# microsoft/SpeechT5

Hardware: AMD Instinct MI355X
Metric: audio-sec/s fwd+bwd SpeechT5-Base (higher is better)
Workload: dtype bf16

## Files before the change

### include/speecht5_hip.h

```cpp
#ifndef SPEECHT5_HIP_H
#define SPEECHT5_HIP_H
#include <stdint.h>
#ifdef __cplusplus
extern "C" {
#endif

#define ST5_F32 0
#define ST5_BF16 1

#define ST5_ACT_NONE 0
#define ST5_ACT_GELU 1
#define ST5_ACT_RELU 2
#define ST5_ACT_TANH 3
#define ST5_ACT_LRELU_01 4
#define ST5_ACT_LRELU_001 5

#define ST5_GEMM_A_KSTRIDED 1
#define ST5_GEMM_B_KSTRIDED 2
#define ST5_GEMM_OUT_F32 4
#define ST5_GEMM_DACT 8
#define ST5_GEMM_DEFERRABLE 16

typedef struct st5_operand {
  const void* ptr;
// ... 44 lines not shown
int st5_gemm_set_mx8_heavy_nk(int nk);
int st5_quant_mxfp8(const void* x, int64_t ld, void* q, int64_t q_ld, uint8_t* s, int64_t s_ld, int64_t rows, int32_t cols, void* stream);
int st5_multi_quant_mxfp8(const void* jobs, int32_t njobs, int32_t nblocks, void* stream);
int st5_gemm_tn_group(const st5_gemm_params* list, int32_t n, int dtype, void* stream);
int st5_gemm_set_tn_group_tile(int mode);
int st5_gemm_tn_group_is_phased(int32_t M, int32_t N, int32_t K);
int st5_gemm_defer_splitk(int enabled, void* stream);
int st5_gemm_flush_splitk(void* stream);

int st5_layernorm_fwd(const void* x, const float* gamma, const float* beta, void* y, float* mean,
                      float* rstd, int64_t rows, int32_t cols, float eps, int dtype, void* stream);
int st5_layernorm_bwd(const void* dy, const void* x, const float* gamma, const float* mean, const float* rstd, void* dx,
                      float* dgamma, float* dbeta, void* ws, int64_t rows, int32_t cols,
                      void* dx_dropped ,
                      float drop_p, uint64_t drop_seed, int dtype, void* stream);
int st5_layernorm_fwd_q8(const void* x, const float* gamma, const float* beta, void* y, float* mean, float* rstd, void* q, uint8_t* sc,
                         int64_t rows, int32_t cols, float eps, void* stream);
int st5_layernorm_bwd_add(const void* dy, const void* x, const float* gamma, const float* mean, const float* rstd, void* dx, float* dgamma,
                          float* dbeta, void* ws, int64_t rows, int32_t cols, const void* addend, int dtype, void* stream);
int st5_layernorm_gelu_fwd(const void* x, const float* gamma, const float* beta, void* y, float* mean, float* rstd, int64_t rows, int32_t cols,
                           float eps, int dtype, void* stream);
int st5_layernorm_gelu_bwd(const void* dy, const void* x, const float* gamma, const float* beta, const float* mean, const float* rstd, void* dx,
                           float* dgamma, float* dbeta, void* ws, int64_t rows, int32_t cols, int dtype, void* stream);
int st5_layernorm_gated_fwd(const void* x, const float* gamma, const float* beta, void* y, float* mean, float* rstd, int64_t rows,
                            int32_t cols, float eps, const float* keep, const void* skip, int dtype, void* stream);
int st5_layernorm_gated_bwd(const void* dy, const void* x, const float* gamma, const float* mean, const float* rstd, void* dx,
                            float* dgamma, float* dbeta, void* ws, int64_t rows, int32_t cols, void* dx_dropped, float drop_p,
                            uint64_t drop_seed, const float* keep, int dtype, void* stream);
int st5_layernorm_fwd_gate(const void* x, const float* gamma, const float* beta, void* y, float* mean, float* rstd, int64_t rows,
                           int32_t cols, float eps, const float* keep, const void* skip, const float* gate, int dtype, void* stream);
int st5_layernorm_bwd_gate(const void* dy, const void* x, const float* gamma, const float* mean, const float* rstd, void* dx, float* dgamma,
                           float* dbeta, void* ws, int64_t rows, int32_t cols, void* dx_dropped, float drop_p, uint64_t drop_seed,
                           const float* keep, const float* gate, int dtype, void* stream);
int st5_layernorm_defer(int enabled, void* stream);
int st5_layernorm_flush(void* stream);
int64_t st5_layernorm_bwd_ws_bytes(int64_t rows, int32_t cols);

int st5_softmax_fwd(const void* scores, const void* qp, const uint8_t* kpm, void* probs, void* probs_drop,
                    int32_t BH, int32_t H, int32_t T, int32_t S, int32_t lds, int32_t nb, int32_t maxrel,
                    int32_t causal, float dropout_p, uint64_t seed, int dtype, void* stream);
int st5_softmax_bwd(void* dP_inout, const void* probs, const float* dP_extra, void* dqp, int32_t BH, int32_t T,
                    int32_t S, int32_t lds, int32_t nb, int32_t maxrel, float dropout_p, uint64_t seed, int dtype,
                    void* stream);

int st5_flash_attn_fwd(const void* q, int64_t q_ld, const void* k, int64_t k_ld, const void* v, int64_t v_ld, void* o,
                       int64_t o_ld, float* lse, const void* pe, const uint8_t* kpm, int32_t B, int32_t H, int32_t T,
                       int32_t S, int32_t head_dim, int32_t nb, int32_t maxrel, int32_t causal, int32_t lds, float scale,
                       float dropout_p, uint64_t seed, int dtype, void* stream);

int32_t st5_flash_attn_qp_row(int32_t nb);
int st5_flash_attn_qp_table(const void* q, int64_t q_ld, const void* pe, void* qp_out, int32_t B, int32_t H, int32_t T, int32_t nb,
                            float scale, int dtype, void* stream);
int st5_flash_attn_set_impl(int impl);

int st5_flash_attn_fwd_qp(const void* q, int64_t q_ld, const void* k, int64_t k_ld, const void* v, int64_t v_ld, void* o,
                          int64_t o_ld, float* lse, const void* pe, const uint8_t* kpm, int32_t B, int32_t H, int32_t T,
                          int32_t S, int32_t head_dim, int32_t nb, int32_t maxrel, int32_t causal, int32_t lds, float scale,
                          float dropout_p, uint64_t seed, void* qp_out, int dtype, void* stream);

int st5_flash_attn_fwd_qp_gate(const void* q, int64_t q_ld, const void* k, int64_t k_ld, const void* v, int64_t v_ld, void* o,
                               int64_t o_ld, float* lse, const void* pe, const uint8_t* kpm, int32_t B, int32_t H, int32_t T,
                               int32_t S, int32_t head_dim, int32_t nb, int32_t maxrel, int32_t causal, int32_t lds, float scale,
                               float dropout_p, uint64_t seed, void* qp_out, const float* gate, int dtype, void* stream);

int st5_flash_attn_bwd(const void* q, int64_t q_ld, const void* k, int64_t k_ld, const void* v, int64_t v_ld, const void* o,
                       int64_t o_ld, const void* dout, int64_t do_ld, void* dq, int64_t dq_ld, void* dk, int64_t dk_ld, void* dv,
                       int64_t dv_ld, const float* lse, float* dvec, const void* pe, const void* qp, void* dqp,
                       const uint8_t* kpm, int32_t B, int32_t H, int32_t T, int32_t S, int32_t head_dim, int32_t nb,
                       int32_t maxrel, int32_t causal, int32_t lds, float scale, float dropout_p, uint64_t seed, int dtype,
                       void* stream);
int st5_flash_attn_bwd_2s(const void* q, int64_t q_ld, const void* k, int64_t k_ld, const void* v, int64_t v_ld, const void* o,
                          int64_t o_ld, const void* dout, int64_t do_ld, void* dq, int64_t dq_ld, void* dk, int64_t dk_ld,
                          void* dv, int64_t dv_ld, const float* lse, float* dvec, const void* pe, const void* qp, void* dqp,
                          const uint8_t* kpm, int32_t B, int32_t H, int32_t T, int32_t S, int32_t head_dim, int32_t nb,
                          int32_t maxrel, int32_t causal, int32_t lds, float scale, float dropout_p, uint64_t seed, int dtype,
                          void* stream, void* stream2);

int st5_flash_attn_bwd_2s_gate(const void* q, int64_t q_ld, const void* k, int64_t k_ld, const void* v, int64_t v_ld, const void* o,
                               int64_t o_ld, const void* dout, int64_t do_ld, void* dq, int64_t dq_ld, void* dk, int64_t dk_ld,
                               void* dv, int64_t dv_ld, const float* lse, float* dvec, const void* pe, const void* qp, void* dqp,
                               const uint8_t* kpm, int32_t B, int32_t H, int32_t T, int32_t S, int32_t head_dim, int32_t nb,
                               int32_t maxrel, int32_t causal, int32_t lds, float scale, float dropout_p, uint64_t seed,
                               const float* gate, int32_t dkv_live, int dtype, void* stream, void* stream2);

int st5_conv0_gn_gelu_fwd(const float* wav, const float* w, const float* gamma, const float* beta, void* out,
                          float* stats, void* ws, int32_t B, int32_t S, int32_t C, int32_t k, int32_t stride,
                          float eps, int dtype, void* stream);
int st5_conv0_gn_gelu_bwd(const float* wav, const float* w, const float* gamma, const float* beta,
                          const float* stats, const void* dY, float* dw, float* dgamma, float* dbeta, void* ws,
                          int32_t B, int32_t S, int32_t C, int32_t k, int32_t stride, float gscale, int dtype,
                          void* stream);
int32_t st5_conv0_mom_count(int32_t k);
int st5_conv0_gn_gelu_fwd_m(const float* wav, const float* w, const float* gamma, const float* beta, void* out, float* stats, double* mom,
                            void* ws, int32_t B, int32_t S, int32_t C, int32_t k, int32_t stride, float eps, int dtype, void* stream);
int st5_conv0_gn_gelu_bwd_m(const float* wav, const float* w, const float* gamma, const float* beta, const float* stats, const double* mom,
                            const void* dY, float* dw, float* dgamma, float* dbeta, void* ws, int32_t B, int32_t S, int32_t C, int32_t k,
                            int32_t stride, float gscale, int dtype, void* stream);
int st5_conv0_gn_gelu_fwd_rows(const float* wav, const int32_t* lens, const float* w, const float* gamma, const float* beta, void* out,
                               float* stats, void* ws, int32_t B, int32_t S, int32_t C, int32_t k, int32_t stride, float eps, int dtype,
                               void* stream);
int st5_conv0_set_mfma(int on);
int st5_conv0_set_fold(int on);
int st5_conv0_set_gelu_table(int on);
int64_t st5_conv0_ws_bytes(int32_t B, int32_t S, int32_t C, int32_t k, int32_t stride);

int st5_cast_from_f32(const float* src, void* dst, int64_t rows, int64_t cols, int32_t transpose, int dtype,
// ... 254 lines not shown
```

### speecht5_amd/csrc/flash_attn2.hip

```cpp
#include "common.h"
#include "../../include/speecht5_hip.h"

#ifndef FA2_ABL
#define FA2_ABL 0
#endif
#ifdef FA2_DMA_NOP
#define FA2_AFTER_DMA(p) asm volatile("s_nop 7\n\ts_nop 7" ::"v"(p) : "memory")
#else
#define FA2_AFTER_DMA(p)
#endif
namespace fa2 {

constexpr int HD = 64;
constexpr int KT = 64;
constexpr int TILE_B = KT * HD * 2;
constexpr int QP_PAD = 8;
constexpr int WIN = 104;
constexpr int WCH = 13;
constexpr int SCR_B = 7168;
constexpr float LOG2E = 1.4426950408889634f;
constexpr float LN2 = 0.6931471805599453f;
constexpr unsigned int PAIR_MUL = 0x9E3779B1u;

typedef __attribute__((address_space(3))) void* lds_ptr_t;
typedef const __attribute__((address_space(1))) void* gbl_ptr_t;
typedef __attribute__((ext_vector_type(4))) short s16x4;
typedef __attribute__((address_space(3))) s16x4* lds_s16x4_ptr;

__device__ __forceinline__ int lds_off(int row, int chunk) { return row * 128 + ((chunk ^ ((row >> 1) & 7)) << 4); }
__device__ __forceinline__ float fast_exp2(float x) { return __builtin_amdgcn_exp2f(x); }

__device__ __forceinline__ void block_coords(int& xb, int& bh) {
  const int nx = (int)gridDim.x, ny = (int)gridDim.y;
  if ((ny & 7) == 0) {
    const int lin = (int)blockIdx.y * nx + (int)blockIdx.x;
    const int per = 8 * nx, grp = lin / per, r = lin - grp * per;
    bh = grp * 8 + (r & 7);
    xb = r >> 3;
  } else {
    xb = (int)blockIdx.x; bh = (int)blockIdx.y;
  }
}

struct TileStager {
  int r[2], lc[2];
  __device__ __forceinline__ void init(int wave, int lane) {
#pragma unroll
    for (int i = 0; i < 2; ++i) {
      r[i] = (i * 4 + wave) * 8 + (lane >> 3);
      lc[i] = ((lane & 7) ^ ((r[i] >> 1) & 7)) * 8;
    }
  }
  __device__ __forceinline__ void issue(const bf16_t* base, long long ld, int row0, int nrows, char* tile, int wave) const {
#pragma unroll
// ... 28 lines not shown
      int c = wbc + (int)(pk[i] & 15u) + 1;
      c = c < 0 ? 0 : (c > nchunks_data + 1 ? nchunks_data + 1 : c);
      const bf16_t* src = qpb + (((pk[i] >> 4) + (unsigned int)c) << 3);
      __builtin_amdgcn_global_load_lds((gbl_ptr_t)src, (lds_ptr_t)(scratch + i * 1024), 16, 0, 0);
      FA2_AFTER_DMA(src);
    }
  }
};

struct TrAddr {
  int sub;
  int colb;
  __device__ __forceinline__ void init(int lane) { sub = (lane & 15) >> 2; colb = 16 * ((lane >> 4) & 1) + 4 * (lane & 3); }
  __device__ __forceinline__ int off(int rbase, int dt) const {
    const int row = rbase + sub, col = 32 * dt + colb;
    return lds_off(row, col >> 3) + (col & 7) * 2;
  }
};
__device__ __forceinline__ bf16x8 tr_frag(const char* tile, int off0, int off1) {
  const s16x4 lo = __builtin_amdgcn_ds_read_tr16_b64_v4i16((lds_s16x4_ptr)(tile + off0));
  const s16x4 hi = __builtin_amdgcn_ds_read_tr16_b64_v4i16((lds_s16x4_ptr)(tile + off1));
  union { struct { s16x4 a, b; } s; bf16x8 v; } u;
  u.s.a = lo; u.s.b = hi;
  return u.v;
}

typedef __attribute__((ext_vector_type(2))) float f32x2_t;
typedef __attribute__((ext_vector_type(2))) __bf16 bf16x2_t;
__device__ __forceinline__ bf16x8 pack8(const f32x16& s, int base) {
  bf16x8 r;
#pragma unroll
  for (int j = 0; j < 4; ++j) {
    const f32x2_t p = {s[base + 2 * j], s[base + 2 * j + 1]};
    const bf16x2_t q = __builtin_convertvector(p, bf16x2_t);
    r[2 * j] = q[0]; r[2 * j + 1] = q[1];
  }
  return r;
}

__device__ __forceinline__ unsigned int kpm_raw(const uint8_t* mrow, int key, int S) {
  return mrow ? (unsigned int)mrow[key < S ? key : S - 1] : 0u;
}

__device__ __forceinline__ void read_bias(unsigned int (&braw)[32], const char* rd) {
  const unsigned short* p = reinterpret_cast<const unsigned short*>(rd);
#if FA2_ABL == 2
  for (int i = 0; i < 32; ++i) { braw[i] = 0x3c00u + i; asm volatile("" : "+v"(braw[i])); }
  return;
#endif
#pragma unroll
  for (int i = 0; i < 32; ++i) {
    const int c = (i >> 4) * 32 + (i & 3) + 8 * ((i & 15) >> 2);
    braw[i] = p[59 - c];
  }
}

template <bool PE_LDS>
__global__ __launch_bounds__(256) void qp_table_kernel(const bf16_t* __restrict__ qg, long long q_ld, const bf16_t* __restrict__ pe,
                                                       bf16_t* __restrict__ qp, int H, int T, int nb, float sc2,
                                                       const float* __restrict__ gate) {
  if (st5_gate_dropped(gate)) return;
  const int tid = threadIdx.x, lane = tid & 63, wave = tid >> 6;
  const int ql = lane & 31, hi = lane >> 5;
  const int bh = blockIdx.y, b = bh / H, h = bh % H;
  const int qi = blockIdx.x * 128 + wave * 32 + ql;
  const int qc = qi < T ? qi : T - 1;
  const int nbp = nb + 2 * QP_PAD;
  bf16x8 qf[4];
#pragma unroll
  for (int ks = 0; ks < 4; ++ks)
    qf[ks] = *reinterpret_cast<const bf16x8*>(qg + ((long long)b * T + qc) * q_ld + h * HD + ks * 16 + hi * 8);
  bf16_t* row = qp + ((long long)bh * T + qc) * nbp + QP_PAD;
  const int nbt = (nb + 31) / 32;
  extern __shared__ __attribute__((aligned(16))) char pe_lds[];
  if (PE_LDS) {
    for (int ch = tid; ch < nb * 8; ch += 256) {
      const int r = ch >> 3, c = ch & 7;
      *reinterpret_cast<u32x4*>(pe_lds + lds_off(r, c)) = *reinterpret_cast<const u32x4*>(pe + r * HD + c * 8);
    }
    __syncthreads();
  }
  const int prow = 16 * ((ql >> 2) & 1) + (ql & 3) + 4 * (ql >> 3);
  for (int bt = 0; bt < nbt; ++bt) {
    int brow = bt * 32 + prow;
    brow = brow < nb ? brow : nb - 1;
    f32x16 acc;
#pragma unroll
    for (int r = 0; r < 16; ++r) acc[r] = 0.f;
#pragma unroll
    for (int ks = 0; ks < 4; ++ks) {
      const bf16x8 pf = PE_LDS ? *reinterpret_cast<const bf16x8*>(pe_lds + lds_off(brow, 2 * ks + hi))
                               : *reinterpret_cast<const bf16x8*>(pe + brow * HD + ks * 16 + hi * 8);
      acc = __builtin_amdgcn_mfma_f32_32x32x16_bf16(pf, qf[ks], acc, 0, 0, 0);
    }
    if (qi < T) {
      const int b0 = bt * 32 + 16 * hi;
#pragma unroll
      for (int u = 0; u < 2; ++u) {
        if (b0 + 8 * u < nb) {
          bf16x8 w;
#pragma unroll
          for (int e = 0; e < 8; ++e) w[e] = (bf16_t)(acc[8 * u + e] * sc2);
          *reinterpret_cast<bf16x8*>(row + b0 + 8 * u) = w;
          if (b0 + 8 * u == 0) {
            const bf16x8 lo = {w[0], w[0], w[0], w[0], w[0], w[0], w[0], w[0]};
            *reinterpret_cast<bf16x8*>(row - 8) = lo;
          }
          if (b0 + 8 * u + 8 == nb) {
            const bf16x8 hv = {w[7], w[7], w[7], w[7], w[7], w[7], w[7], w[7]};
            *reinterpret_cast<bf16x8*>(row + nb) = hv;
          }
        }
      }
    }
  }
}

struct Args {
  const bf16_t* q; const bf16_t* k; const bf16_t* v; bf16_t* o; float* lse;
  const bf16_t* qp;
  const uint8_t* kpm;
  long long q_ld, k_ld, v_ld, o_ld;
  int B, H, T, S, nb, maxrel, causal, lds;
  float scale, dropout_p;
  unsigned long long seed;
  const float* gate;
};

template <int BMODE , bool MASK>
__device__ __forceinline__ float tile_scores(f32x16& s0, f32x16& s1, float sc2, const unsigned int (&braw)[32], float buni,
                                             unsigned long long km, int jrel) {
  float tmax = -INFINITY;
#pragma unroll
  for (int t = 0; t < 2; ++t) {
#pragma unroll
    for (int r = 0; r < 16; ++r) {
      const int c = t * 32 + (r & 3) + 8 * (r >> 2);
      const float b = BMODE == 1 ? __uint_as_float(braw[16 * t + r] << 16) : (BMODE == 2 ? buni : 0.f);
      float x = fmaf(t == 0 ? s0[r] : s1[r], sc2, b);
      if (MASK) { if (((km >> c) & 1ull) || c > jrel) x = -INFINITY; }
      if (t == 0) s0[r] = x; else s1[r] = x;
      tmax = fmaxf(tmax, x);
    }
  }
  return tmax;
}

template <bool DROP>
__device__ __forceinline__ float tile_probs(f32x16& s0, f32x16& s1, float m_use, unsigned int key32, unsigned int hoff, unsigned int thresh) {
  float psum = 0.f;
#pragma unroll
  for (int t = 0; t < 2; ++t) {
#pragma unroll
    for (int g = 0; g < 4; ++g) {
      unsigned int bits0 = 0u, bits1 = 0u;
      if (DROP) {
        bits0 = drop_pair_bits_pc(key32, (unsigned int)(16 * t + 4 * g) * PAIR_MUL + hoff);
        bits1 = drop_pair_bits_pc(key32, (unsigned int)(16 * t + 4 * g + 1) * PAIR_MUL + hoff);
      }
#pragma unroll
      for (int e = 0; e < 4; ++e) {
        const int r = 4 * g + e;
        float p = fast_exp2((t == 0 ? s0[r] : s1[r]) - m_use);
        psum += p;
        if (DROP) p = drop_keep(e < 2 ? bits0 : bits1, e & 1, thresh) ? p : 0.f;
        if (t == 0) s0[r] = p; else s1[r] = p;
      }
    }
  }
  return psum;
}

struct WinGeom { int mode; int wbc; int mis; };
__device__ __forceinline__ WinGeom win_geom(int qw0, int j0, int maxrel, int nb) {
  WinGeom g;
  const int bmin = qw0 - (j0 + 63) + maxrel, bmax = qw0 + 31 - j0 + maxrel;
  g.mode = bmax <= 0 ? 1 : (bmin >= nb - 1 ? 2 : 0);
#if FA2_ABL == 4
  g.mode = g.mode == 0 ? 1 : g.mode;
#endif
  const int wb8 = bmin & ~7;
  g.wbc = wb8 >> 3;
  g.mis = bmin - wb8;
  return g;
}

template <bool BIAS, bool DROP>
__global__ __launch_bounds__(256, 2) void fwd_kernel(const Args a) {
  if (st5_gate_dropped(a.gate)) return;
#ifdef FA2_PAD256
  ST5_PAD_TO_256_VGPRS();
#endif
  extern __shared__ __attribute__((aligned(16))) char smem[];
  char* kbuf = smem;
  char* vbuf = smem + 2 * TILE_B;
  const int tid = threadIdx.x, lane = tid & 63;
  const int wave = __builtin_amdgcn_readfirstlane(tid >> 6);
  char* scratch = smem + 4 * TILE_B + wave * SCR_B;
  const int ql = lane & 31, hi = lane >> 5;
  int xb_, bh;
  block_coords(xb_, bh);
  const int b = bh / a.H, h = bh % a.H;
  const int qblk = xb_ * 128;
  const int qw0 = qblk + wave * 32;
  const int qi = qw0 + ql;
  const int qc = qi < a.T ? qi : a.T - 1;
  const bool qvalid = qi < a.T;

  bf16x8 qf[4];
#pragma unroll
  for (int ks = 0; ks < 4; ++ks)
    qf[ks] = *reinterpret_cast<const bf16x8*>(a.q + ((long long)b * a.T + qc) * a.q_ld + h * HD + ks * 16 + hi * 8);

  int nkeys = a.S;
  if (a.causal) {
    const int qmax = (qblk + 127 < a.T ? qblk + 127 : a.T - 1) + (a.S - a.T);
    nkeys = qmax + 1 < a.S ? qmax + 1 : a.S;
  }
  const int ntiles = (nkeys + KT - 1) / KT;

  const bf16_t* kbase = a.k + (long long)b * a.S * a.k_ld + h * HD;
  const bf16_t* vbase = a.v + (long long)b * a.S * a.v_ld + h * HD;
  TileStager ts;
  ts.init(wave, lane);
  const int nbp = a.nb + 2 * QP_PAD;
  const bf16_t* qpb = BIAS ? a.qp + (long long)bh * a.T * nbp : nullptr;
  WinStager wsg;
  if (BIAS) wsg.init(lane, qw0, a.T, nbp);
  float blo = 0.f, bhi = 0.f;
  if (BIAS) {
    blo = (float)qpb[(long long)qc * nbp];
    bhi = (float)qpb[(long long)qc * nbp + QP_PAD + a.nb];
  }
  TrAddr tra;
  tra.init(lane);
  int voff[2][2];
#pragma unroll
  for (int dt = 0; dt < 2; ++dt) {
    voff[dt][0] = tra.off(4 * hi, dt);
    voff[dt][1] = tra.off(8 + 4 * hi, dt);
  }

  const uint8_t* mrow = a.kpm ? a.kpm + (long long)b * a.S : nullptr;
  unsigned int raw_next = kpm_raw(mrow, lane, a.S);

  ts.issue(kbase, a.k_ld, 0, a.S, kbuf, wave);
  ts.issue(vbase, a.v_ld, 0, a.S, vbuf, wave);
  WinGeom wg = BIAS ? win_geom(qw0, 0, a.maxrel, a.nb) : WinGeom{0, 0, 0};
  if (BIAS && wg.mode == 0) wsg.issue(qpb, wg.wbc, a.nb >> 3, scratch);

  f32x16 o0, o1;
#pragma unroll
  for (int r = 0; r < 16; ++r) { o0[r] = 0.f; o1[r] = 0.f; }
  float m_run = -INFINITY, l_run = 0.f;
  constexpr bool drop = DROP;
  const unsigned int thresh = drop ? dropout_thresh(a.dropout_p) : 0u;
  const unsigned int seedf = drop ? drop_seed_fold(a.seed) : 0u;
  const float inv_keep = drop ? 1.f / (1.f - a.dropout_p) : 1.f;
  const float sc2 = a.scale * LOG2E;
  const int jmax = a.causal ? qi + (a.S - a.T) : 0x3fffffff;
  const unsigned long long ctr_blk = ((unsigned long long)bh * a.T + (unsigned long long)qc) * (unsigned long long)(drop_row_stride(a.lds) >> 6);
  const unsigned int hoff = hi ? 2u * PAIR_MUL : 0u;
  const int rd_lane = (ql * WIN + ql + 4 - 4 * hi) * 2;

  for (int jt = 0; jt < ntiles; ++jt) {
    const char* kt = kbuf + (jt & 1) * TILE_B;
    const char* vt = vbuf + (jt & 1) * TILE_B;
    const int j0 = jt * KT;
    asm volatile("s_waitcnt vmcnt(0)" ::: "memory");
    __builtin_amdgcn_s_barrier();
    const unsigned long long kmask = __ballot(raw_next != 0u || j0 + lane >= a.S);
    bf16x8 kfa[4], kfb[4];
#pragma unroll
    for (int ks = 0; ks < 4; ++ks) {
      kfa[ks] = *reinterpret_cast<const bf16x8*>(kt + lds_off(ql, 2 * ks + hi));
      kfb[ks] = *reinterpret_cast<const bf16x8*>(kt + lds_off(32 + ql, 2 * ks + hi));
    }
    unsigned int braw[32];
// ... 691 lines not shown
          const int bk0 = q0 - ki + a.maxrel;
          int voff = (q0 * a.nb + bk0) * 2;
          int estride2 = dqp_estride2;
          asm volatile("" : "+v"(voff), "+s"(estride2));
          const int bmin = qs0 - (kw0 + 31) + a.maxrel, bmax = qs0 + 31 - kw0 + a.maxrel;
          if (bmin > 0 && bmax < a.nb - 1 && kw0 + 31 < a.S && qs0 + 31 < a.T) {
            dkv_store_dqp<true>(df, dqp_rsrc, voff, 0, 0, estride2);
          } else {
            const int cmax = a.nb - 1 - bk0 < a.T - q0 ? a.nb - 1 - bk0 : a.T - q0;
            dkv_store_dqp<false>(df, dqp_rsrc, voff, kvalid ? -bk0 : 32, cmax, estride2);
          }
        }
      }
    }
    if (qt + 1 < nqt) side_store(smem + ((qt + 1) & 1) * QBUF_B);
  }
  if (kvalid) {
    bf16_t* krow = a.dk + ((long long)b * a.S + ki) * a.dk_ld + h * HD;
    bf16_t* vrow = a.dv + ((long long)b * a.S + ki) * a.dv_ld + h * HD;
#pragma unroll
    for (int dt = 0; dt < 2; ++dt)
#pragma unroll
      for (int g = 0; g < 4; ++g) {
        bf16x4 wk, wv;
#pragma unroll
        for (int e = 0; e < 4; ++e) {
          wk[e] = (bf16_t)((dt == 0 ? dk0[4 * g + e] : dk1[4 * g + e]) * a.scale);
          wv[e] = (bf16_t)(dt == 0 ? dv0[4 * g + e] : dv1[4 * g + e]);
        }
        *reinterpret_cast<bf16x4*>(krow + dt * 32 + 8 * g + 4 * hi) = wk;
        *reinterpret_cast<bf16x4*>(vrow + dt * 32 + 8 * g + 4 * hi) = wv;
      }
  }
}

}

extern "C" {
int st5_flash1_attn_fwd_qp(const void* q, int64_t q_ld, const void* k, int64_t k_ld, const void* v, int64_t v_ld, void* o, int64_t o_ld,
                           float* lse, const void* pe, const uint8_t* kpm, int32_t B, int32_t H, int32_t T, int32_t S, int32_t head_dim,
                           int32_t nb, int32_t maxrel, int32_t causal, int32_t lds, float scale, float dropout_p, uint64_t seed,
                           void* qp_out, int dtype, void* stream);
int st5_flash1_attn_bwd_2s(const void* q, int64_t q_ld, const void* k, int64_t k_ld, const void* v, int64_t v_ld, const void* o,
                           int64_t o_ld, const void* dout, int64_t do_ld, void* dq, int64_t dq_ld, void* dk, int64_t dk_ld, void* dv,
                           int64_t dv_ld, const float* lse, float* dvec, const void* pe, const void* qp, void* dqp, const uint8_t* kpm,
                           int32_t B, int32_t H, int32_t T, int32_t S, int32_t head_dim, int32_t nb, int32_t maxrel, int32_t causal,
                           int32_t lds, float scale, float dropout_p, uint64_t seed, int dtype, void* stream, void* stream2);
int st5_stream_fork(void* from_stream, void* to_stream);
}

namespace {
int g_impl = 2;
bool g_attr = false;
int set_attrs() {
  if (g_attr) return ST5_OK;
  const void* fns[] = {(const void*)fa2::fwd_kernel<true, true>, (const void*)fa2::fwd_kernel<false, true>, (const void*)fa2::fwd_kernel<true, false>,
                       (const void*)fa2::fwd_kernel<false, false>, (const void*)fa2::bwd_dq_kernel<true, true>, (const void*)fa2::bwd_dq_kernel<false, true>,
                       (const void*)fa2::bwd_dq_kernel<true, false>, (const void*)fa2::bwd_dq_kernel<false, false>, (const void*)fa2::bwd_dkv_kernel<true, true>,
                       (const void*)fa2::bwd_dkv_kernel<false, true>, (const void*)fa2::bwd_dkv_kernel<true, false>, (const void*)fa2::bwd_dkv_kernel<false, false>};
  for (const void* f : fns)
#ifdef FA2_DKV_FAT_LDS
    if (hipFuncSetAttribute(f, hipFuncAttributeMaxDynamicSharedMemorySize, 128 * 1024) != hipSuccess) return ST5_ERR_LAUNCH;
#else
    if (hipFuncSetAttribute(f, hipFuncAttributeMaxDynamicSharedMemorySize, 96 * 1024) != hipSuccess) return ST5_ERR_LAUNCH;
#endif
  g_attr = true;
  return ST5_OK;
}
}

extern "C" int st5_flash_attn_set_impl(int impl) {
  if (impl != 1 && impl != 2) return ST5_ERR_ARG;
  g_impl = impl;
  return ST5_OK;
}
extern "C" int32_t st5_flash_attn_qp_row(int32_t nb) { return g_impl == 2 ? nb + 2 * fa2::QP_PAD : nb; }

static int qp_table(const void* q, int64_t q_ld, const void* pe, void* qp_out, int32_t B, int32_t H, int32_t T, int32_t nb, float scale,
                    int dtype, void* stream, const float* gate) {
  if (!q || !pe || !qp_out || B <= 0 || H <= 0 || T <= 0 || nb <= 0 || nb % 8 || dtype != ST5_BF16 || q_ld % 8) return ST5_ERR_ARG;
  const size_t pe_bytes = (size_t)nb * fa2::HD * 2;
  if (pe_bytes <= 64 * 1024) {
    static bool attr = false;
    if (!attr) {
      if (hipFuncSetAttribute((const void*)fa2::qp_table_kernel<true>, hipFuncAttributeMaxDynamicSharedMemorySize, 64 * 1024) != hipSuccess) return ST5_ERR_LAUNCH;
      attr = true;
    }
    hipLaunchKernelGGL(fa2::qp_table_kernel<true>, dim3((T + 127) / 128, B * H), dim3(256), pe_bytes, (hipStream_t)stream, (const bf16_t*)q,
                       (long long)q_ld, (const bf16_t*)pe, (bf16_t*)qp_out, H, T, nb, scale * fa2::LOG2E, gate);
  } else {
    hipLaunchKernelGGL(fa2::qp_table_kernel<false>, dim3((T + 127) / 128, B * H), dim3(256), 0, (hipStream_t)stream, (const bf16_t*)q,
                       (long long)q_ld, (const bf16_t*)pe, (bf16_t*)qp_out, H, T, nb, scale * fa2::LOG2E, gate);
  }
  HIP_CHECK_LAUNCH();
  return ST5_OK;
}
extern "C" int st5_flash_attn_qp_table(const void* q, int64_t q_ld, const void* pe, void* qp_out, int32_t B, int32_t H, int32_t T,
                                       int32_t nb, float scale, int dtype, void* stream) {
  return qp_table(q, q_ld, pe, qp_out, B, H, T, nb, scale, dtype, stream, nullptr);
}

extern "C" int st5_flash_attn_fwd_qp_gate(const void* q, int64_t q_ld, const void* k, int64_t k_ld, const void* v, int64_t v_ld, void* o,
                                          int64_t o_ld, float* lse, const void* pe, const uint8_t* kpm, int32_t B, int32_t H, int32_t T,
                                          int32_t S, int32_t head_dim, int32_t nb, int32_t maxrel, int32_t causal, int32_t lds, float scale,
                                          float dropout_p, uint64_t seed, void* qp_out, const float* gate, int dtype, void* stream) {
  if (gate && (g_impl == 1 || (pe && !qp_out))) return ST5_ERR_ARG;
  if (g_impl == 1 || (pe && !qp_out))
    return st5_flash1_attn_fwd_qp(q, q_ld, k, k_ld, v, v_ld, o, o_ld, lse, pe, kpm, B, H, T, S, head_dim, nb, maxrel, causal, lds, scale,
                                  dropout_p, seed, g_impl == 1 ? qp_out : nullptr, dtype, stream);
  if (!q || !k || !v || !o || B <= 0 || H <= 0 || T <= 0 || S <= 0) return ST5_ERR_ARG;
  if (dtype != ST5_BF16 || head_dim != fa2::HD) return ST5_ERR_ARG;
  if (q_ld % 8 || k_ld % 8 || v_ld % 8 || o_ld % 4) return ST5_ERR_ALIGN;
  if (pe && (nb != 2 * maxrel || nb % 8 || nb > 1024)) return ST5_ERR_ARG;
  if ((long long)B * H * T * (pe ? nb + 16 : 1) >= (1ll << 31)) return ST5_ERR_ARG;
  if (set_attrs() != ST5_OK) return ST5_ERR_LAUNCH;
  hipStream_t s = (hipStream_t)stream;
  if (pe) {
    const int rc = qp_table(q, q_ld, pe, qp_out, B, H, T, nb, scale, dtype, stream, gate);
    if (rc) return rc;
  }
  fa2::Args a;
  a.gate = gate;
  a.q = (const bf16_t*)q; a.k = (const bf16_t*)k; a.v = (const bf16_t*)v; a.o = (bf16_t*)o; a.lse = lse;
  a.qp = pe ? (const bf16_t*)qp_out : nullptr; a.kpm = kpm;
  a.q_ld = q_ld; a.k_ld = k_ld; a.v_ld = v_ld; a.o_ld = o_ld;
  a.B = B; a.H = H; a.T = T; a.S = S; a.nb = pe ? nb : 0; a.maxrel = maxrel; a.causal = causal; a.lds = lds;
  a.scale = scale; a.dropout_p = dropout_p; a.seed = seed;
  dim3 grid((T + 127) / 128, B * H), block(256);
  const bool dr = dropout_p > 0.f;
  const size_t shm = (size_t)4 * fa2::TILE_B + (pe ? 4 * fa2::SCR_B : 0);
  if (pe && dr) hipLaunchKernelGGL((fa2::fwd_kernel<true, true>), grid, block, shm, s, a);
  else if (pe) hipLaunchKernelGGL((fa2::fwd_kernel<true, false>), grid, block, shm, s, a);
  else if (dr) hipLaunchKernelGGL((fa2::fwd_kernel<false, true>), grid, block, shm, s, a);
  else hipLaunchKernelGGL((fa2::fwd_kernel<false, false>), grid, block, shm, s, a);
  HIP_CHECK_LAUNCH();
  return ST5_OK;
}

extern "C" int st5_flash_attn_fwd_qp(const void* q, int64_t q_ld, const void* k, int64_t k_ld, const void* v, int64_t v_ld, void* o,
                                     int64_t o_ld, float* lse, const void* pe, const uint8_t* kpm, int32_t B, int32_t H, int32_t T,
                                     int32_t S, int32_t head_dim, int32_t nb, int32_t maxrel, int32_t causal, int32_t lds, float scale,
                                     float dropout_p, uint64_t seed, void* qp_out, int dtype, void* stream) {
  return st5_flash_attn_fwd_qp_gate(q, q_ld, k, k_ld, v, v_ld, o, o_ld, lse, pe, kpm, B, H, T, S, head_dim, nb, maxrel, causal, lds, scale,
                                    dropout_p, seed, qp_out, nullptr, dtype, stream);
}

extern "C" int st5_flash_attn_fwd(const void* q, int64_t q_ld, const void* k, int64_t k_ld, const void* v, int64_t v_ld, void* o,
                                  int64_t o_ld, float* lse, const void* pe, const uint8_t* kpm, int32_t B, int32_t H, int32_t T, int32_t S,
                                  int32_t head_dim, int32_t nb, int32_t maxrel, int32_t causal, int32_t lds, float scale, float dropout_p,
                                  uint64_t seed, int dtype, void* stream) {
  return st5_flash_attn_fwd_qp(q, q_ld, k, k_ld, v, v_ld, o, o_ld, lse, pe, kpm, B, H, T, S, head_dim, nb, maxrel, causal, lds, scale,
                               dropout_p, seed, nullptr, dtype, stream);
}

extern "C" int st5_flash_attn_bwd_2s_gate(const void* q, int64_t q_ld, const void* k, int64_t k_ld, const void* v, int64_t v_ld, const void* o,
                                          int64_t o_ld, const void* dout, int64_t do_ld, void* dq, int64_t dq_ld, void* dk, int64_t dk_ld,
                                          void* dv, int64_t dv_ld, const float* lse, float* dvec, const void* pe, const void* qp, void* dqp,
                                          const uint8_t* kpm, int32_t B, int32_t H, int32_t T, int32_t S, int32_t head_dim, int32_t nb,
                                          int32_t maxrel, int32_t causal, int32_t lds, float scale, float dropout_p, uint64_t seed,
                                          const float* gate, int32_t dkv_live, int dtype, void* stream, void* stream2) {
  if (gate && g_impl == 1) return ST5_ERR_ARG;
  if (g_impl == 1)
    return st5_flash1_attn_bwd_2s(q, q_ld, k, k_ld, v, v_ld, o, o_ld, dout, do_ld, dq, dq_ld, dk, dk_ld, dv, dv_ld, lse, dvec, pe, qp, dqp,
                                  kpm, B, H, T, S, head_dim, nb, maxrel, causal, lds, scale, dropout_p, seed, dtype, stream, stream2);
  if (!q || !k || !v || !o || !dout || !dq || !dk || !dv || !lse || !dvec || B <= 0 || H <= 0 || T <= 0 || S <= 0) return ST5_ERR_ARG;
  if (dtype != ST5_BF16 || head_dim != fa2::HD) return ST5_ERR_ARG;
  if (q_ld % 8 || k_ld % 8 || v_ld % 8 || o_ld % 8 || do_ld % 8 || dq_ld % 4 || dk_ld % 4 || dv_ld % 4) return ST5_ERR_ALIGN;
  if (pe && (!qp || !dqp || nb != 2 * maxrel || nb % 8 || nb > 1024)) return ST5_ERR_ARG;
  if (pe && (reinterpret_cast<uintptr_t>(dqp) % 16) != 0) return ST5_ERR_ALIGN;
  if ((long long)B * H * T * (pe ? nb + 16 : 1) >= (1ll << 31)) return ST5_ERR_ARG;
  if (set_attrs() != ST5_OK) return ST5_ERR_LAUNCH;
  fa2::BwdArgs a;
  a.gate = gate; a.dkv_live = dkv_live;
  a.q = (const bf16_t*)q; a.k = (const bf16_t*)k; a.v = (const bf16_t*)v; a.o = (const bf16_t*)o; a.dout = (const bf16_t*)dout;
  a.dq = (bf16_t*)dq; a.dk = (bf16_t*)dk; a.dv = (bf16_t*)dv; a.lse = lse; a.dvec = dvec;
  a.qp = pe ? (const bf16_t*)qp : nullptr; a.dqp = (bf16_t*)dqp; a.kpm = kpm;
  a.q_ld = q_ld; a.k_ld = k_ld; a.v_ld = v_ld; a.o_ld = o_ld; a.do_ld = do_ld; a.dq_ld = dq_ld; a.dk_ld = dk_ld; a.dv_ld = dv_ld;
  a.B = B; a.H = H; a.T = T; a.S = S; a.nb = pe ? nb : 0; a.maxrel = maxrel; a.causal = causal; a.lds = lds;
  a.scale = scale; a.dropout_p = dropout_p; a.seed = seed;
  hipStream_t s = (hipStream_t)stream, s2 = (hipStream_t)stream2;
  const long long rows = (long long)B * H * T;
  a.dvec_in_dq = (s2 == nullptr || s2 == s) ? 1 : 0;
  if (pe && !a.dvec_in_dq && hipMemsetAsync(dqp, 0, (size_t)B * H * T * nb * 2, s) != hipSuccess) return ST5_ERR_LAUNCH;
// ... 49 lines not shown
```

### speecht5_amd/hip.py

```python
import ctypes
import os
from ctypes import POINTER, Structure, byref, c_char_p, c_double, c_float, c_int, c_int32, c_int64, c_uint64, c_void_p

import torch

F32, BF16 = 0, 1
ACT_NONE, ACT_GELU, ACT_RELU, ACT_TANH, ACT_LRELU_01, ACT_LRELU_001 = 0, 1, 2, 3, 4, 5
A_KSTRIDED, B_KSTRIDED, OUT_F32, DACT = 1, 2, 4, 8
DEFERRABLE = 16

_LIB_PATH = os.environ.get("ST5_HIP_LIB") or os.path.join(os.path.dirname(os.path.abspath(__file__)), "libspeecht5_hip.so")


class HipLibraryMissing(RuntimeError):
    pass


class HipKernelError(RuntimeError):
    pass


class Operand(Structure):
    _fields_ = [("ptr", c_void_p), ("ld", c_int64), ("rpb", c_int32), ("seg", c_int32),
                ("bstride", c_int64), ("seg_stride", c_int64), ("zs0", c_int64), ("zs1", c_int64)]
# ... 18 lines not shown
    "st5_gemm_set_mx8_tile": (c_int, [c_int]),
    "st5_gemm_set_mx8_heavy_nk": (c_int, [c_int]),
    "st5_gemm_set_tn_group_tile": (c_int, [c_int]),
    "st5_gemm_tn_group_is_phased": (c_int, [c_int32, c_int32, c_int32]),
    "st5_gemm_set_splitk_target": (c_int, [c_int]),
    "st5_gemm_set_deep_ring": (c_int, [c_int, c_int]),
    "st5_gemm_set_nt_slots": (c_int, [c_int]),
    "st5_gemm_tn_group": (c_int, [c_void_p, c_int32, c_int, c_void_p]),
    "st5_gemm_defer_splitk": (c_int, [c_int, c_void_p]),
    "st5_gemm_flush_splitk": (c_int, [c_void_p]),
    "st5_layernorm_fwd": (c_int, [c_void_p, c_void_p, c_void_p, c_void_p, c_void_p, c_void_p, c_int64, c_int32,
                                  c_float, c_int, c_void_p]),
    "st5_layernorm_bwd": (c_int, [c_void_p, c_void_p, c_void_p, c_void_p, c_void_p, c_void_p, c_void_p, c_void_p, c_void_p,
                                  c_int64, c_int32, c_void_p, c_float, c_uint64, c_int, c_void_p]),
    "st5_layernorm_gated_fwd": (c_int, [c_void_p, c_void_p, c_void_p, c_void_p, c_void_p, c_void_p, c_int64, c_int32,
                                        c_float, c_void_p, c_void_p, c_int, c_void_p]),
    "st5_layernorm_gated_bwd": (c_int, [c_void_p, c_void_p, c_void_p, c_void_p, c_void_p, c_void_p, c_void_p, c_void_p, c_void_p,
                                        c_int64, c_int32, c_void_p, c_float, c_uint64, c_void_p, c_int, c_void_p]),
    "st5_layernorm_fwd_gate": (c_int, [c_void_p, c_void_p, c_void_p, c_void_p, c_void_p, c_void_p, c_int64, c_int32,
                                       c_float, c_void_p, c_void_p, c_void_p, c_int, c_void_p]),
    "st5_layernorm_bwd_gate": (c_int, [c_void_p, c_void_p, c_void_p, c_void_p, c_void_p, c_void_p, c_void_p, c_void_p, c_void_p,
                                       c_int64, c_int32, c_void_p, c_float, c_uint64, c_void_p, c_void_p, c_int, c_void_p]),
    "st5_colsum_ws_gate": (c_int, [c_void_p, c_void_p, c_void_p, c_int64, c_int32, c_int64, c_float, c_int32, c_void_p, c_int,
                                   c_void_p]),
    "st5_flash_attn_fwd_qp_gate": (c_int, [c_void_p, c_int64, c_void_p, c_int64, c_void_p, c_int64, c_void_p, c_int64, c_void_p, c_void_p,
                                           c_void_p, c_int32, c_int32, c_int32, c_int32, c_int32, c_int32, c_int32, c_int32, c_int32,
                                           c_float, c_float, c_uint64, c_void_p, c_void_p, c_int, c_void_p]),
    "st5_flash_attn_bwd_2s_gate": (c_int, [c_void_p, c_int64, c_void_p, c_int64, c_void_p, c_int64, c_void_p, c_int64, c_void_p, c_int64,
                                           c_void_p, c_int64, c_void_p, c_int64, c_void_p, c_int64, c_void_p, c_void_p, c_void_p, c_void_p,
                                           c_void_p, c_void_p, c_int32, c_int32, c_int32, c_int32, c_int32, c_int32, c_int32, c_int32,
                                           c_int32, c_float, c_float, c_uint64, c_void_p, c_int32, c_int, c_void_p, c_void_p]),
    "st5_layernorm_defer": (c_int, [c_int, c_void_p]),
    "st5_layernorm_flush": (c_int, [c_void_p]),
    "st5_layernorm_bwd_ws_bytes": (c_int64, [c_int64, c_int32]),
    "st5_softmax_fwd": (c_int, [c_void_p, c_void_p, c_void_p, c_void_p, c_void_p, c_int32, c_int32, c_int32, c_int32,
                                c_int32, c_int32, c_int32, c_int32, c_float, c_uint64, c_int, c_void_p]),
    "st5_softmax_bwd": (c_int, [c_void_p, c_void_p, c_void_p, c_void_p, c_int32, c_int32, c_int32, c_int32, c_int32,
                                c_int32, c_float, c_uint64, c_int, c_void_p]),
    "st5_flash_attn_fwd": (c_int, [c_void_p, c_int64, c_void_p, c_int64, c_void_p, c_int64, c_void_p, c_int64, c_void_p, c_void_p,
                                   c_void_p, c_int32, c_int32, c_int32, c_int32, c_int32, c_int32, c_int32, c_int32, c_int32,
                                   c_float, c_float, c_uint64, c_int, c_void_p]),
    "st5_flash_attn_fwd_qp": (c_int, [c_void_p, c_int64, c_void_p, c_int64, c_void_p, c_int64, c_void_p, c_int64, c_void_p, c_void_p,
                                      c_void_p, c_int32, c_int32, c_int32, c_int32, c_int32, c_int32, c_int32, c_int32, c_int32,
                                      c_float, c_float, c_uint64, c_void_p, c_int, c_void_p]),
    "st5_flash_attn_bwd_2s": (c_int, [c_void_p, c_int64, c_void_p, c_int64, c_void_p, c_int64, c_void_p, c_int64, c_void_p, c_int64,
                                      c_void_p, c_int64, c_void_p, c_int64, c_void_p, c_int64, c_void_p, c_void_p, c_void_p, c_void_p,
                                      c_void_p, c_void_p, c_int32, c_int32, c_int32, c_int32, c_int32, c_int32, c_int32, c_int32,
                                      c_int32, c_float, c_float, c_uint64, c_int, c_void_p, c_void_p]),
    "st5_flash_attn_bwd": (c_int, [c_void_p, c_int64, c_void_p, c_int64, c_void_p, c_int64, c_void_p, c_int64, c_void_p, c_int64,
                                   c_void_p, c_int64, c_void_p, c_int64, c_void_p, c_int64, c_void_p, c_void_p, c_void_p, c_void_p,
                                   c_void_p, c_void_p, c_int32, c_int32, c_int32, c_int32, c_int32, c_int32, c_int32, c_int32,
                                   c_int32, c_float, c_float, c_uint64, c_int, c_void_p]),
    "st5_flash_attn_set_impl": (c_int, [c_int]),
    "st5_gemm_set_tn_phased": (c_int, [c_int]),
    "st5_gemm_mxfp8": (c_int, [POINTER(GemmParams), c_void_p, c_int64, c_void_p, c_int64, c_void_p]),
    "st5_quant_mxfp8": (c_int, [c_void_p, c_int64, c_void_p, c_int64, c_void_p, c_int64, c_int64, c_int32, c_void_p]),
    "st5_multi_quant_mxfp8": (c_int, [c_void_p, c_int32, c_int32, c_void_p]),
    "st5_gemm_mxfp8_q": (c_int, [POINTER(GemmParams), c_void_p, c_int64, c_void_p, c_int64, c_void_p, c_int64, c_void_p, c_int64, c_void_p]),
    "st5_layernorm_bwd_add": (c_int, [c_void_p, c_void_p, c_void_p, c_void_p, c_void_p, c_void_p, c_void_p, c_void_p, c_void_p, c_int64, c_int32,
                                      c_void_p, c_int, c_void_p]),
    "st5_layernorm_gelu_fwd": (c_int, [c_void_p, c_void_p, c_void_p, c_void_p, c_void_p, c_void_p, c_int64, c_int32, c_float, c_int, c_void_p]),
    "st5_layernorm_gelu_bwd": (c_int, [c_void_p, c_void_p, c_void_p, c_void_p, c_void_p, c_void_p, c_void_p, c_void_p, c_void_p, c_void_p,
                                       c_int64, c_int32, c_int, c_void_p]),
    "st5_layernorm_fwd_q8": (c_int, [c_void_p, c_void_p, c_void_p, c_void_p, c_void_p, c_void_p, c_void_p, c_void_p, c_int64, c_int32, c_float,
                                     c_void_p]),
    "st5_flash_attn_qp_row": (c_int32, [c_int32]),
    "st5_flash_attn_qp_table": (c_int, [c_void_p, c_int64, c_void_p, c_void_p, c_int32, c_int32, c_int32, c_int32, c_float, c_int, c_void_p]),
    "st5_conv0_gn_gelu_fwd": (c_int, [c_void_p, c_void_p, c_void_p, c_void_p, c_void_p, c_void_p, c_void_p, c_int32,
                                      c_int32, c_int32, c_int32, c_int32, c_float, c_int, c_void_p]),
    "st5_conv0_gn_gelu_bwd": (c_int, [c_void_p, c_void_p, c_void_p, c_void_p, c_void_p, c_void_p, c_void_p, c_void_p,
                                      c_void_p, c_void_p, c_int32, c_int32, c_int32, c_int32, c_int32, c_float, c_int,
                                      c_void_p]),
    "st5_conv0_gn_gelu_fwd_m": (c_int, [c_void_p, c_void_p, c_void_p, c_void_p, c_void_p, c_void_p, c_void_p, c_void_p, c_int32,
                                        c_int32, c_int32, c_int32, c_int32, c_float, c_int, c_void_p]),
    "st5_conv0_gn_gelu_bwd_m": (c_int, [c_void_p, c_void_p, c_void_p, c_void_p, c_void_p, c_void_p, c_void_p, c_void_p, c_void_p,
                                        c_void_p, c_void_p, c_int32, c_int32, c_int32, c_int32, c_int32, c_float, c_int,
                                        c_void_p]),
    "st5_conv0_gn_gelu_fwd_rows": (c_int, [c_void_p, c_void_p, c_void_p, c_void_p, c_void_p, c_void_p, c_void_p, c_void_p, c_int32,
                                           c_int32, c_int32, c_int32, c_int32, c_float, c_int, c_void_p]),
    "st5_conv0_mom_count": (c_int32, [c_int32]),
    "st5_conv0_ws_bytes": (c_int64, [c_int32, c_int32, c_int32, c_int32, c_int32]),
    "st5_conv0_set_mfma": (c_int, [c_int]),
    "st5_conv0_set_fold": (c_int, [c_int]),
    "st5_conv0_set_gelu_table": (c_int, [c_int]),
    "st5_cast_from_f32": (c_int, [c_void_p, c_void_p, c_int64, c_int64, c_int32, c_int, c_void_p]),
    "st5_cast_to_f32": (c_int, [c_void_p, c_void_p, c_int64, c_int, c_void_p]),
    "st5_colsum_ws": (c_int, [c_void_p, c_void_p, c_void_p, c_int64, c_int32, c_int64, c_float, c_int32, c_int,
                              c_void_p]),
    "st5_colsum_ws_bytes": (c_int64, [c_int64, c_int32]),
    "st5_relpos_bwd": (c_int, [c_void_p, c_void_p, c_int64, c_void_p, c_void_p, c_int64, c_void_p, c_int32, c_int32, c_int32, c_int32,
                               c_float, c_void_p, c_int, c_void_p]),
    "st5_relpos_bwd_supported": (c_int, [c_int32]),
    "st5_relpos_dpe_final": (c_int, [c_void_p, c_void_p, c_int64, c_int32, c_void_p, c_int, c_void_p]),
    "st5_sumsq": (c_int, [c_void_p, c_void_p, c_int64, c_float, c_int32, c_int, c_void_p]),
    "st5_axpby": (c_int, [c_void_p, c_void_p, c_int64, c_float, c_float, c_int, c_void_p]),
    "st5_select": (c_int, [c_void_p, c_void_p, c_void_p, c_void_p, c_int64, c_void_p]),
    "st5_select_bwd": (c_int, [c_void_p, c_void_p, c_void_p, c_void_p, c_int64, c_void_p]),
    "st5_skip_grad": (c_int, [c_void_p, c_void_p, c_void_p, c_int64, c_void_p]),
    "st5_act_fwd": (c_int, [c_void_p, c_void_p, c_int64, c_int32, c_int, c_void_p]),
    "st5_act_bwd": (c_int, [c_void_p, c_void_p, c_void_p, c_int64, c_int32, c_int, c_void_p]),
    "st5_channel_affine": (c_int, [c_void_p, c_void_p, c_void_p, c_void_p, c_int64, c_int32, c_int32, c_int, c_void_p]),
    "st5_dropout": (c_int, [c_void_p, c_void_p, c_int64, c_float, c_uint64, c_int, c_void_p]),
    "st5_masked_fill_rows": (c_int, [c_void_p, c_void_p, c_void_p, c_int64, c_int32, c_int, c_void_p]),
    "st5_masked_fill_rows_bwd": (c_int, [c_void_p, c_void_p, c_void_p, c_int64, c_int32, c_int, c_void_p]),
    "st5_add_table_rows": (c_int, [c_void_p, c_void_p, c_void_p, c_void_p, c_int64, c_int32, c_float, c_int,
                                   c_void_p]),
    "st5_add_table_rows_dev": (c_int, [c_void_p, c_void_p, c_void_p, c_void_p, c_int64, c_int32, c_void_p, c_int, c_void_p]),
# ... 388 lines not shown
```

Baseline: 3108.

## Compute relative-position qp table inline inside flash attention forward kernel

Moves the q·pe relative-position bias table computation into the flash-attention forward kernel's prologue instead of launching a separate qp_table kernel. Each block stages the pe matrix into shared memory with the tile stager, writes its own qp rows, then fences and syncs before the main loop reads them through the window stager. This removes one kernel launch and the separate pass over q, at the cost of a longer prologue and an extra barrier in every forward block. The behaviour is gated by an environment knob and is on by default. The standalone qp_table kernel also switches to DMA staging of pe.

```diff
diff --git a/include/speecht5_hip.h b/include/speecht5_hip.h
--- a/include/speecht5_hip.h
+++ b/include/speecht5_hip.h
@@ -120,6 +120,7 @@
 int st5_flash_attn_qp_table(const void* q, int64_t q_ld, const void* pe, void* qp_out, int32_t B, int32_t H, int32_t T, int32_t nb,
                             float scale, int dtype, void* stream);
 int st5_flash_attn_set_impl(int impl);
+int st5_flash_attn_set_qp_inline(int on);
 
 int st5_flash_attn_fwd_qp(const void* q, int64_t q_ld, const void* k, int64_t k_ld, const void* v, int64_t v_ld, void* o,
                           int64_t o_ld, float* lse, const void* pe, const uint8_t* kpm, int32_t B, int32_t H, int32_t T,
diff --git a/speecht5_amd/csrc/flash_attn2.hip b/speecht5_amd/csrc/flash_attn2.hip
--- a/speecht5_amd/csrc/flash_attn2.hip
+++ b/speecht5_amd/csrc/flash_attn2.hip
@@ -1,5 +1,6 @@
 #include "common.h"
 #include "../../include/speecht5_hip.h"
+#include <cstdlib>
 
 #ifndef FA2_ABL
 #define FA2_ABL 0
@@ -134,6 +135,55 @@
   for (int i = 0; i < 32; ++i) {
     const int c = (i >> 4) * 32 + (i & 3) + 8 * ((i & 15) >> 2);
     braw[i] = p[59 - c];
+  }
+}
+
+template <bool PE_LDS>
+__device__ __forceinline__ void qp_rows(const bf16x8 (&qf)[4], const bf16_t* __restrict__ pe, char* pe_lds, bf16_t* row, bool qvalid,
+                                        int nb, float sc2, int tid, int ql, int hi) {
+  const int nbt = (nb + 31) / 32;
+  if (PE_LDS) {
+    const int lane = tid & 63, wave = __builtin_amdgcn_readfirstlane(tid >> 6);
+    TileStager ts;
+    ts.init(wave, lane);
+    for (int t = 0; t * KT < nb; ++t) ts.issue(pe, HD, t * KT, nb, pe_lds + t * TILE_B, wave);
+    asm volatile("s_waitcnt vmcnt(0)" ::: "memory");
+    __syncthreads();
+  }
+  const int prow = 16 * ((ql >> 2) & 1) + (ql & 3) + 4 * (ql >> 3);
+#pragma unroll 2
+  for (int bt = 0; bt < nbt; ++bt) {
+    int brow = bt * 32 + prow;
+    brow = brow < nb ? brow : nb - 1;
+    f32x16 acc;
+#pragma unroll
+    for (int r = 0; r < 16; ++r) acc[r] = 0.f;
+#pragma unroll
+    for (int ks = 0; ks < 4; ++ks) {
+      const bf16x8 pf = PE_LDS ? *reinterpret_cast<const bf16x8*>(pe_lds + lds_off(brow, 2 * ks + hi))
+                               : *reinterpret_cast<const bf16x8*>(pe + brow * HD + ks * 16 + hi * 8);
+      acc = __builtin_amdgcn_mfma_f32_32x32x16_bf16(pf, qf[ks], acc, 0, 0, 0);
+    }
+    if (qvalid) {
+      const int b0 = bt * 32 + 16 * hi;
+#pragma unroll
+      for (int u = 0; u < 2; ++u) {
+        if (b0 + 8 * u < nb) {
+          bf16x8 w;
+#pragma unroll
+          for (int e = 0; e < 8; ++e) w[e] = (bf16_t)(acc[8 * u + e] * sc2);
+          *reinterpret_cast<bf16x8*>(row + b0 + 8 * u) = w;
+          if (b0 + 8 * u == 0) {
+            const bf16x8 lo = {w[0], w[0], w[0], w[0], w[0], w[0], w[0], w[0]};
+            *reinterpret_cast<bf16x8*>(row - 8) = lo;
+          }
+          if (b0 + 8 * u + 8 == nb) {
+            const bf16x8 hv = {w[7], w[7], w[7], w[7], w[7], w[7], w[7], w[7]};
+            *reinterpret_cast<bf16x8*>(row + nb) = hv;
+          }
+        }
+      }
+    }
   }
 }
 
@@ -152,55 +202,14 @@
 #pragma unroll
   for (int ks = 0; ks < 4; ++ks)
     qf[ks] = *reinterpret_cast<const bf16x8*>(qg + ((long long)b * T + qc) * q_ld + h * HD + ks * 16 + hi * 8);
-  bf16_t* row = qp + ((long long)bh * T + qc) * nbp + QP_PAD;
-  const int nbt = (nb + 31) / 32;
   extern __shared__ __attribute__((aligned(16))) char pe_lds[];
-  if (PE_LDS) {
-    for (int ch = tid; ch < nb * 8; ch += 256) {
-      const int r = ch >> 3, c = ch & 7;
-      *reinterpret_cast<u32x4*>(pe_lds + lds_off(r, c)) = *reinterpret_cast<const u32x4*>(pe + r * HD + c * 8);
-    }
-    __syncthreads();
-  }
-  const int prow = 16 * ((ql >> 2) & 1) + (ql & 3) + 4 * (ql >> 3);
-  for (int bt = 0; bt < nbt; ++bt) {
-    int brow = bt * 32 + prow;
-    brow = brow < nb ? brow : nb - 1;
-    f32x16 acc;
-#pragma unroll
-    for (int r = 0; r < 16; ++r) acc[r] = 0.f;
-#pragma unroll
-    for (int ks = 0; ks < 4; ++ks) {
-      const bf16x8 pf = PE_LDS ? *reinterpret_cast<const bf16x8*>(pe_lds + lds_off(brow, 2 * ks + hi))
-                               : *reinterpret_cast<const bf16x8*>(pe + brow * HD + ks * 16 + hi * 8);
-      acc = __builtin_amdgcn_mfma_f32_32x32x16_bf16(pf, qf[ks], acc, 0, 0, 0);
-    }
-    if (qi < T) {
-      const int b0 = bt * 32 + 16 * hi;
-#pragma unroll
-      for (int u = 0; u < 2; ++u) {
-        if (b0 + 8 * u < nb) {
-          bf16x8 w;
-#pragma unroll
-          for (int e = 0; e < 8; ++e) w[e] = (bf16_t)(acc[8 * u + e] * sc2);
-          *reinterpret_cast<bf16x8*>(row + b0 + 8 * u) = w;
-          if (b0 + 8 * u == 0) {
-            const bf16x8 lo = {w[0], w[0], w[0], w[0], w[0], w[0], w[0], w[0]};
-            *reinterpret_cast<bf16x8*>(row - 8) = lo;
-          }
-          if (b0 + 8 * u + 8 == nb) {
-            const bf16x8 hv = {w[7], w[7], w[7], w[7], w[7], w[7], w[7], w[7]};
-            *reinterpret_cast<bf16x8*>(row + nb) = hv;
-          }
-        }
-      }
-    }
-  }
+  qp_rows<PE_LDS>(qf, pe, pe_lds, qp + ((long long)bh * T + qc) * nbp + QP_PAD, qi < T, nb, sc2, tid, ql, hi);
 }
 
 struct Args {
   const bf16_t* q; const bf16_t* k; const bf16_t* v; bf16_t* o; float* lse;
   const bf16_t* qp;
+  const bf16_t* pe;
   const uint8_t* kpm;
   long long q_ld, k_ld, v_ld, o_ld;
   int B, H, T, S, nb, maxrel, causal, lds;
@@ -294,6 +303,15 @@
   for (int ks = 0; ks < 4; ++ks)
     qf[ks] = *reinterpret_cast<const bf16x8*>(a.q + ((long long)b * a.T + qc) * a.q_ld + h * HD + ks * 16 + hi * 8);
 
+  const int nbp = a.nb + 2 * QP_PAD;
+  if (BIAS && a.pe) {
+    qp_rows<true>(qf, a.pe, smem, const_cast<bf16_t*>(a.qp) + ((long long)bh * a.T + qc) * nbp + QP_PAD, qvalid, a.nb, a.scale * LOG2E,
+                  tid, ql, hi);
+    __builtin_amdgcn_fence(__ATOMIC_RELEASE, "workgroup");
+    __syncthreads();
+    __builtin_amdgcn_fence(__ATOMIC_ACQUIRE, "workgroup");
+  }
+
   int nkeys = a.S;
   if (a.causal) {
     const int qmax = (qblk + 127 < a.T ? qblk + 127 : a.T - 1) + (a.S - a.T);
@@ -305,7 +323,6 @@
   const bf16_t* vbase = a.v + (long long)b * a.S * a.v_ld + h * HD;
   TileStager ts;
   ts.init(wave, lane);
-  const int nbp = a.nb + 2 * QP_PAD;
   const bf16_t* qpb = BIAS ? a.qp + (long long)bh * a.T * nbp : nullptr;
   WinStager wsg;
   if (BIAS) wsg.init(lane, qw0, a.T, nbp);
@@ -1103,6 +1120,14 @@
 namespace {
 int g_impl = 2;
 bool g_attr = false;
+int g_qp_inline = -1;
+int knob(int& g, const char* env) {
+  if (g < 0) {
+    const char* e = std::getenv(env);
+    g = (e && e[0] == '0' && e[1] == '\0') ? 0 : 1;
+  }
+  return g;
+}
 int set_attrs() {
   if (g_attr) return ST5_OK;
   const void* fns[] = {(const void*)fa2::fwd_kernel<true, true>, (const void*)fa2::fwd_kernel<false, true>, (const void*)fa2::fwd_kernel<true, false>,
@@ -1125,7 +1150,14 @@
   g_impl = impl;
   return ST5_OK;
 }
+extern "C" int st5_flash_attn_set_qp_inline(int on) {
+  if (on != 0 && on != 1) return ST5_ERR_ARG;
+  g_qp_inline = on;
+  return ST5_OK;
+}
 extern "C" int32_t st5_flash_attn_qp_row(int32_t nb) { return g_impl == 2 ? nb + 2 * fa2::QP_PAD : nb; }
+
+static size_t pe_image_bytes(int32_t nb) { return (size_t)((nb + fa2::KT - 1) / fa2::KT) * fa2::TILE_B; }
 
 static int qp_table(const void* q, int64_t q_ld, const void* pe, void* qp_out, int32_t B, int32_t H, int32_t T, int32_t nb, float scale,
                     int dtype, void* stream, const float* gate) {
@@ -1137,7 +1169,7 @@
       if (hipFuncSetAttribute((const void*)fa2::qp_table_kernel<true>, hipFuncAttributeMaxDynamicSharedMemorySize, 64 * 1024) != hipSuccess) return ST5_ERR_LAUNCH;
       attr = true;
     }
-    hipLaunchKernelGGL(fa2::qp_table_kernel<true>, dim3((T + 127) / 128, B * H), dim3(256), pe_bytes, (hipStream_t)stream, (const bf16_t*)q,
+    hipLaunchKernelGGL(fa2::qp_table_kernel<true>, dim3((T + 127) / 128, B * H), dim3(256), pe_image_bytes(nb), (hipStream_t)stream, (const bf16_t*)q,
                        (long long)q_ld, (const bf16_t*)pe, (bf16_t*)qp_out, H, T, nb, scale * fa2::LOG2E, gate);
   } else {
     hipLaunchKernelGGL(fa2::qp_table_kernel<false>, dim3((T + 127) / 128, B * H), dim3(256), 0, (hipStream_t)stream, (const bf16_t*)q,
@@ -1166,12 +1198,15 @@
   if ((long long)B * H * T * (pe ? nb + 16 : 1) >= (1ll << 31)) return ST5_ERR_ARG;
   if (set_attrs() != ST5_OK) return ST5_ERR_LAUNCH;
   hipStream_t s = (hipStream_t)stream;
-  if (pe) {
+  const size_t shm = (size_t)4 * fa2::TILE_B + (pe ? 4 * fa2::SCR_B : 0);
+  const bool qp_inline = pe && knob(g_qp_inline, "ST5_FA2_QP_INLINE") && pe_image_bytes(nb) <= shm;
+  if (pe && !qp_inline) {
     const int rc = qp_table(q, q_ld, pe, qp_out, B, H, T, nb, scale, dtype, stream, gate);
     if (rc) return rc;
   }
   fa2::Args a;
   a.gate = gate;
+  a.pe = qp_inline ? (const bf16_t*)pe : nullptr;
   a.q = (const bf16_t*)q; a.k = (const bf16_t*)k; a.v = (const bf16_t*)v; a.o = (bf16_t*)o; a.lse = lse;
   a.qp = pe ? (const bf16_t*)qp_out : nullptr; a.kpm = kpm;
   a.q_ld = q_ld; a.k_ld = k_ld; a.v_ld = v_ld; a.o_ld = o_ld;
@@ -1179,7 +1214,6 @@
   a.scale = scale; a.dropout_p = dropout_p; a.seed = seed;
   dim3 grid((T + 127) / 128, B * H), block(256);
   const bool dr = dropout_p > 0.f;
-  const size_t shm = (size_t)4 * fa2::TILE_B + (pe ? 4 * fa2::SCR_B : 0);
   if (pe && dr) hipLaunchKernelGGL((fa2::fwd_kernel<true, true>), grid, block, shm, s, a);
   else if (pe) hipLaunchKernelGGL((fa2::fwd_kernel<true, false>), grid, block, shm, s, a);
   else if (dr) hipLaunchKernelGGL((fa2::fwd_kernel<false, true>), grid, block, shm, s, a);
diff --git a/speecht5_amd/hip.py b/speecht5_amd/hip.py
--- a/speecht5_amd/hip.py
+++ b/speecht5_amd/hip.py
@@ -94,7 +94,7 @@
                                    c_void_p, c_void_p, c_int32, c_int32, c_int32, c_int32, c_int32, c_int32, c_int32, c_int32,
                                    c_int32, c_float, c_float, c_uint64, c_int, c_void_p]),
     "st5_flash_attn_set_impl": (c_int, [c_int]),
-    "st5_gemm_set_tn_phased": (c_int, [c_int]),
+    "st5_flash_attn_set_qp_inline": (c_int, [c_int]),    "st5_gemm_set_tn_phased": (c_int, [c_int]),
     "st5_gemm_mxfp8": (c_int, [POINTER(GemmParams), c_void_p, c_int64, c_void_p, c_int64, c_void_p]),
     "st5_quant_mxfp8": (c_int, [c_void_p, c_int64, c_void_p, c_int64, c_void_p, c_int64, c_int64, c_int32, c_void_p]),
     "st5_multi_quant_mxfp8": (c_int, [c_void_p, c_int32, c_int32, c_void_p]),
```

Measured after the change: 3120, median of 6. About the same (+0.4%).
